# Youncy-Hu/MAGE

Hardware: AMD Instinct MI355X
Metric: generated frames/sec (64x64, 16-frame clips) (higher is better)
Workload: dtype bf16

## Files before the change

### include/mage_hip_ext.h

```cpp
#ifndef MAGE_HIP_EXT_H
#define MAGE_HIP_EXT_H

#include "mage_hip.h"

#ifdef __cplusplus
extern "C" {
#endif

int mage_token_stats(const float* logits, int64_t rows, int32_t K, int64_t ld, int64_t group, int64_t in_group_stride, int64_t in_off,
                     const int64_t* tokens, int64_t tok_group_stride, int64_t tok_off, float temperature, int32_t top_k, float top_p,
                     float* policy_logprob, float* policy_entropy, int32_t* kept, float* entropy, void* stream);

int mage_policy_loss(const float* logits, int64_t rows, int32_t K, int64_t ld, const int64_t* tokens, const float* advantage, int64_t adv_div,
                     const float* behaviour_logprob, float temperature, int32_t top_k, float top_p, float clip_lo, float clip_hi,
                     float entropy_coef, float* row_loss, float* logprob, float* entropy, uint32_t* cut, float* summary, void* stream);
int mage_policy_loss_bwd(const float* logits, int64_t rows, int32_t K, int64_t ld, const int64_t* tokens, const float* advantage,
                         int64_t adv_div, const float* behaviour_logprob, const uint32_t* cut, float temperature, float clip_lo,
                         float clip_hi, float entropy_coef, const float* grad_out, void* dlogits, int32_t dl_dtype, void* stream);

int mage_policy_loss_anchored(const float* logits, int64_t rows, int32_t K, int64_t ld, const int64_t* tokens, const float* advantage,
                              int64_t adv_div, const float* behaviour_logprob, const float* reference_logprob, float temperature,
                              int32_t top_k, float top_p, float clip_lo, float clip_hi, float entropy_coef, float kl_coef, float* row_loss,
                              float* logprob, float* entropy, uint32_t* cut, float* kl, float* summary, void* stream);
int mage_policy_loss_anchored_bwd(const float* logits, int64_t rows, int32_t K, int64_t ld, const int64_t* tokens, const float* advantage,
                                  int64_t adv_div, const float* behaviour_logprob, const float* reference_logprob, const uint32_t* cut,
                                  float temperature, float clip_lo, float clip_hi, float entropy_coef, float kl_coef, const float* grad_out,
                                  void* dlogits, int32_t dl_dtype, void* stream);

int mage_sumsq(const float* g, int64_t n, double* out, void* stream);
int mage_adam_clipped(float* p, const float* g, float* m, float* v, int64_t n, float lr, float beta1, float beta2, float eps, int32_t step,
                      float grad_scale, const double* sumsq, float max_norm, float* norm_out, void* stream);

int mage_video_metrics(const float* video, int64_t video_clip_stride, const float* target, int64_t target_clip_stride, int64_t clips, int32_t T,
                       int32_t C, int32_t H, int32_t W, int64_t tgt_div, float data_range, float* mse, float* psnr, float* ssim, void* stream);

int mage_group_advantages(const float* frame_reward, int64_t groups, int32_t N, int32_t T, int32_t mode, float eps, float* reward,
                          float* advantage, void* stream);

int mage_frame_advantages(const float* frame_reward, int64_t groups, int32_t N, int32_t T, float gamma, int32_t mode, float eps, int32_t slots,
                          int32_t slot_off, float* returns, float* advantage, void* stream);

int mage_video_noise(const int64_t* seeds, int64_t B, int32_t C, int64_t hw, float* nchw, float* rows, void* stream);

int mage_guide_logits(const float* cond, const float* uncond, float* out, int64_t rows, int32_t K, int64_t ld, int64_t group,
                      int64_t in_group_stride, int64_t in_off, const float* scale, int64_t scale_div, void* stream);

int mage_preference_loss(const float* clip_logprob, const float* reference_logprob, int64_t clips, const int64_t* pairs, int64_t n_pairs,
                         float beta, float label_smoothing, int32_t mode, float* pair_loss, float* pair_margin, float* clip_coef,
                         float* summary, void* stream);

int mage_token_logprob_bwd(const float* logits, int64_t rows, int32_t K, int64_t ld, const int64_t* tokens, const float* weight,
                           int64_t weight_div, const float* grad_out, void* dlogits, int32_t dl_dtype, void* stream);

int mage_gemm_attn_fused_qkv(const mage_gemm_desc* desc, int32_t axis, float scale, void* stream);
int mage_gemm_attn_fused_qkv_kernel_name(const mage_gemm_desc* desc, int32_t axis, char* buf, int32_t len);

int mage_apply_known_tokens(int64_t* tokens, int64_t rows, int64_t group, int64_t tok_group_stride, int64_t tok_off, const int64_t* known,
                            int64_t known_group_stride, int64_t known_off, int64_t known_clip_div, int32_t K, float* logprob,
                            float* policy_logprob, float* entropy, float* policy_entropy, int32_t* kept, void* stream);

int mage_policy_loss_masked(const float* logits, int64_t rows, int32_t K, int64_t ld, const int64_t* tokens, const float* advantage,
                            int64_t adv_div, const float* behaviour_logprob, const float* reference_logprob, float temperature, int32_t top_k,
                            float top_p, float clip_lo, float clip_hi, float entropy_coef, float kl_coef, float* row_loss, float* logprob,
                            float* entropy, uint32_t* cut, float* kl, float* summary, float* norm, const uint8_t* given, void* stream);
int mage_policy_loss_masked_bwd(const float* logits, int64_t rows, int32_t K, int64_t ld, const int64_t* tokens, const float* advantage,
                                int64_t adv_div, const float* behaviour_logprob, const float* reference_logprob, const uint32_t* cut,
                                float temperature, float clip_lo, float clip_hi, float entropy_coef, float kl_coef, const float* grad_out,
                                const float* norm, void* dlogits, int32_t dl_dtype, const uint8_t* given, void* stream);

int mage_policy_loss_grouped(const float* logits, int64_t rows, int32_t K, int64_t ld, const int64_t* tokens, const float* advantage,
                             int64_t adv_div, const float* behaviour_logprob, const float* reference_logprob, float temperature, int32_t top_k,
                             float top_p, float clip_lo, float clip_hi, float entropy_coef, float kl_coef, float* row_loss, float* logprob,
                             float* entropy, uint32_t* cut, float* kl, float* summary, float* norm, const uint8_t* given, int64_t ratio_div,
                             float* group_logratio, int32_t* group_count, void* stream);
int mage_policy_loss_grouped_bwd(const float* logits, int64_t rows, int32_t K, int64_t ld, const int64_t* tokens, const float* advantage,
                                 int64_t adv_div, const float* behaviour_logprob, const float* reference_logprob, const uint32_t* cut,
                                 float temperature, float clip_lo, float clip_hi, float entropy_coef, float kl_coef, const float* grad_out,
                                 const float* norm, void* dlogits, int32_t dl_dtype, const uint8_t* given, int64_t ratio_div,
                                 const float* group_logratio, void* stream);

int mage_token_logprob_bwd_masked(const float* logits, int64_t rows, int32_t K, int64_t ld, const int64_t* tokens, const float* weight,
                                  int64_t weight_div, const float* grad_out, void* dlogits, int32_t dl_dtype, const uint8_t* given,
                                  void* stream);

int mage_distill_loss(const float* logits, int64_t rows, int32_t K, int64_t ld, const float* teacher, int64_t ld_t, float temperature,
                      int32_t mode, const uint8_t* given, float* row_kl, float* summary, float* norm, void* stream);
int mage_distill_loss_bwd(const float* logits, int64_t rows, int32_t K, int64_t ld, const float* teacher, int64_t ld_t, float temperature,
                          int32_t mode, const uint8_t* given, const float* row_kl, const float* grad_out, const float* norm, void* dlogits,
                          int32_t dl_dtype, void* stream);
// ... 6 lines not shown
```

### mage_amd/_lib.py

```python
from __future__ import annotations

import ctypes as C
import os
from typing import Optional

_HERE = os.path.dirname(os.path.abspath(__file__))
LIB_PATH = os.environ.get("MAGE_HIP_LIB", os.path.join(_HERE, "lib", "libmage_hip.so"))

F32, BF16, BF16X3, F16X3, F16 = 0, 1, 2, 3, 4
ACT_NONE, ACT_RELU, ACT_QUICKGELU, ACT_GELU_ERF, ACT_TANH, ACT_QUICKGELU_GRAD = 0, 1, 2, 3, 4, 5
ABI_VERSION = 10

i32, i64, f32, vp = C.c_int32, C.c_int64, C.c_float, C.c_void_p


class GemmDesc(C.Structure):
    _fields_ = [
        ("dtype", i32), ("M", i32), ("N", i32), ("K", i32),
        ("A", vp), ("W", vp), ("Y", vp),
        ("lda", i32), ("ldy", i32), ("y_dtype", i32),
        ("out_h", i32), ("out_w", i32), ("in_h", i32), ("in_w", i32),
        ("a_img_stride", i32), ("a_off", i32),
        ("taps_h", i32), ("taps_w", i32), ("cin", i32), ("stride", i32),
        ("dy0", i32), ("dx0", i32), ("dys", i32), ("dxs", i32),
# ... 79 lines not shown
    "mage_colsum": (C.c_int, [vp, i64, i64, i32, vp, i32, vp]),
    "mage_row_sum": (C.c_int, [vp, i32, i64, i64, i32, vp, i32, vp]),
    "mage_sum_partials": (C.c_int, [vp, i64, i32, i64, vp, i32, vp]),
    "mage_layernorm_bwd": (C.c_int, [vp, vp, vp, i32, vp, vp, i32, i64, i32, f32, i32, vp, f32, C.c_uint64, vp]),
    "mage_act": (C.c_int, [vp, vp, i32, i64, i32, vp]),
    "mage_act_bwd": (C.c_int, [vp, vp, vp, i32, i64, i32, vp]),
    "mage_cross_entropy_bwd": (C.c_int, [vp, vp, i64, i32, vp, vp, i32, vp]),
    "mage_embedding_bwd": (C.c_int, [vp, vp, i32, vp, i64, i32, i32, i64, i64, i64, i64, vp, i64, vp]),
    "mage_group_rowsum": (C.c_int, [vp, i32, i64, i32, i64, i64, vp, i64, vp, i32, vp]),
    "mage_attention_bwd": (C.c_int, [C.POINTER(AttnDesc), vp, vp, vp, vp, i32, i32, i32, vp]),
    "mage_dropout": (C.c_int, [vp, i32, vp, i32, i64, f32, C.c_uint64, i32, vp]),
    "mage_dropout_add": (C.c_int, [vp, i32, vp, vp, vp, i64, f32, C.c_uint64, vp]),
    "mage_dropout_add_layernorm": (C.c_int, [vp, i32, vp, vp, vp, vp, vp, i32, i64, i32, f32, f32, C.c_uint64, vp]),
    "mage_adam": (C.c_int, [vp, vp, vp, vp, i64, f32, f32, f32, f32, i32, f32, vp]),
}

EXT_SIGNATURES = {
    "mage_token_stats": (C.c_int, [vp, i64, i32, i64, i64, i64, i64, vp, i64, i64, f32, i32, f32, vp, vp, vp, vp, vp]),
    "mage_policy_loss": (C.c_int, [vp, i64, i32, i64, vp, vp, i64, vp, f32, i32, f32, f32, f32, f32, vp, vp, vp, vp, vp, vp]),
    "mage_policy_loss_bwd": (C.c_int, [vp, i64, i32, i64, vp, vp, i64, vp, vp, f32, f32, f32, f32, vp, vp, i32, vp]),
    "mage_policy_loss_anchored": (C.c_int, [vp, i64, i32, i64, vp, vp, i64, vp, vp, f32, i32, f32, f32, f32, f32, f32, vp, vp, vp, vp, vp, vp, vp]),
    "mage_policy_loss_anchored_bwd": (C.c_int, [vp, i64, i32, i64, vp, vp, i64, vp, vp, vp, f32, f32, f32, f32, f32, vp, vp, i32, vp]),
    "mage_sumsq": (C.c_int, [vp, i64, vp, vp]),
    "mage_adam_clipped": (C.c_int, [vp, vp, vp, vp, i64, f32, f32, f32, f32, i32, f32, vp, f32, vp, vp]),
    "mage_video_metrics": (C.c_int, [vp, i64, vp, i64, i64, i32, i32, i32, i32, i64, f32, vp, vp, vp, vp]),
    "mage_group_advantages": (C.c_int, [vp, i64, i32, i32, i32, f32, vp, vp, vp]),
    "mage_frame_advantages": (C.c_int, [vp, i64, i32, i32, f32, i32, f32, i32, i32, vp, vp, vp]),
    "mage_video_noise": (C.c_int, [vp, i64, i32, i64, vp, vp, vp]),
    "mage_guide_logits": (C.c_int, [vp, vp, vp, i64, i32, i64, i64, i64, i64, vp, i64, vp]),
    "mage_preference_loss": (C.c_int, [vp, vp, i64, vp, i64, f32, f32, i32, vp, vp, vp, vp, vp]),
    "mage_token_logprob_bwd": (C.c_int, [vp, i64, i32, i64, vp, vp, i64, vp, vp, i32, vp]),
    "mage_gemm_attn_fused_qkv": (C.c_int, [C.POINTER(GemmDesc), i32, f32, vp]),
    "mage_gemm_attn_fused_qkv_kernel_name": (C.c_int, [C.POINTER(GemmDesc), i32, C.c_char_p, i32]),
    "mage_apply_known_tokens": (C.c_int, [vp, i64, i64, i64, i64, vp, i64, i64, i64, i32, vp, vp, vp, vp, vp, vp]),
    "mage_policy_loss_masked": (C.c_int, [vp, i64, i32, i64, vp, vp, i64, vp, vp, f32, i32, f32, f32, f32, f32, f32, vp, vp, vp, vp, vp, vp, vp,
                                          vp, vp]),
    "mage_policy_loss_masked_bwd": (C.c_int, [vp, i64, i32, i64, vp, vp, i64, vp, vp, vp, f32, f32, f32, f32, f32, vp, vp, vp, i32, vp, vp]),
    "mage_policy_loss_grouped": (C.c_int, [vp, i64, i32, i64, vp, vp, i64, vp, vp, f32, i32, f32, f32, f32, f32, f32, vp, vp, vp, vp, vp, vp, vp,
                                           vp, i64, vp, vp, vp]),
    "mage_policy_loss_grouped_bwd": (C.c_int, [vp, i64, i32, i64, vp, vp, i64, vp, vp, vp, f32, f32, f32, f32, f32, vp, vp, vp, i32, vp, i64, vp,
                                               vp]),
    "mage_token_logprob_bwd_masked": (C.c_int, [vp, i64, i32, i64, vp, vp, i64, vp, vp, i32, vp, vp]),
    "mage_distill_loss": (C.c_int, [vp, i64, i32, i64, vp, i64, f32, i32, vp, vp, vp, vp, vp]),
    "mage_distill_loss_bwd": (C.c_int, [vp, i64, i32, i64, vp, i64, f32, i32, vp, vp, vp, vp, vp, i32, vp]),
}

_lib: Optional[C.CDLL] = None
_inited_devices = set()


class MageHipError(RuntimeError):
    pass


def load(path: str = LIB_PATH) -> C.CDLL:
    global _lib
    if _lib is not None:
        return _lib
    if not os.path.exists(path):
        raise MageHipError(
            f"{path} not found: the HIP extension is not built. Run `python -c 'import __graft_entry__ as g; g.build()'` "
            f"(or `make -C mage_amd/csrc`). There is no CPU/PyTorch fallback for the MAGE product path.")
    import torch
    lib = C.CDLL(path)
    for name, (res, args) in {**SIGNATURES, **EXT_SIGNATURES}.items():
        fn = getattr(lib, name)
# ... 24 lines not shown
```

### mage_amd/config.py

```python
from __future__ import annotations

import contextlib
import dataclasses
import os
from typing import Iterator

__all__ = ["Config", "ENV", "get", "override", "lib_option", "lib_options", "lib_flag", "LIB_OPTIONS"]


@dataclasses.dataclass(frozen=True)
class Config:
    qk_fuse: bool = True
    ln_fold: bool = True
    stream_16bit: bool = True
    attn_split: bool = True
    frame_table: bool = True
    auto_graph: bool = True
    encode_split: bool = True
    decode_table: bool = True
    decode_split: bool = True
    decode_taps8: bool = True
    decode_resblock_fusion: bool = True
    decode_head_fusion: bool = True
    decode_phase_merge: bool = True
    decode_relu_fold: bool = True
    train_f32_branch: bool = False
    train_wgrad_transpose: bool = False
    train_emit: bool = True
    train_dual: bool = True
    train_taps: bool = True
    train_enc_split: bool = True


ENV = {
    "ln_fold": ("MAGE_NO_LN_FOLD", False),
    "qk_fuse": ("MAGE_NO_QK_FUSE", False),
    "stream_16bit": ("MAGE_STREAM_FP32", False),
    "attn_split": ("MAGE_ATTN_SPLIT_FP32", False),
    "frame_table": ("MAGE_NO_FRAME_TABLE", False),
    "auto_graph": ("MAGE_NO_AUTO_GRAPH", False),
    "encode_split": ("MAGE_ENCODE_FP32", False),
    "decode_table": ("MAGE_NO_DECODE_TABLE", False),
    "decode_split": ("MAGE_DECODE_FP32", False),
    "decode_taps8": ("MAGE_DECODE_NO_TAPS8", False),
    "decode_resblock_fusion": ("MAGE_DECODE_NO_RESBLOCK_FUSION", False),
    "decode_head_fusion": ("MAGE_DECODE_NO_HEAD_FUSION", False),
    "decode_phase_merge": ("MAGE_DECODE_NO_PHASE_MERGE", False),
    "decode_relu_fold": ("MAGE_DECODE_NO_RELU_FOLD", False),
    "train_f32_branch": ("MAGE_TRAIN_F32_BRANCH", True),
    "train_wgrad_transpose": ("MAGE_WGRAD_TRANSPOSE", True),
    "train_emit": ("MAGE_TRAIN_NO_EMIT", False),
    "train_dual": ("MAGE_TRAIN_NO_DUAL", False),
    "train_taps": ("MAGE_TRAIN_NO_TAPS", False),
    "train_enc_split": ("MAGE_TRAIN_ENC_FP32", False),
}

LIB_OPTIONS = ("gemm_no_4w", "gemm_no_4h", "gemm_4h_plain", "gemm4_train_forms", "gemm_no_8phase", "gemm_no_taps8", "gemm_no_narrow", "gemm_no_narrow_few", "gemm_no_small",
               "gemm_small_m", "gemm_stagger_groups", "gemm_stagger_percent", "gemm_stagger_forced",
               "gemm4_stagger_groups", "gemm4_stagger_percent", "attn_no_mfma", "attn_no_fewq", "vq_no_mfma", "conv_no_tile")


def _set(v) -> bool:
    return bool(v) and v != "0"


def _from_env() -> Config:
    kw = {}
    for field, (var, when_set) in ENV.items():
        if _set(os.environ.get(var)):
# ... 74 lines not shown
```

### mage_amd/modules/mage_model.py

```python
from __future__ import annotations

import contextlib
import ctypes
import gc
import math
from collections import OrderedDict
from math import exp
from typing import Dict, Optional, Tuple

import torch
from torch import nn

from .. import config, ops
from ..utils.util import default, instantiate_from_config, zero_module
from .vqvae_model import VectorQuantizedVAE, _Derived, _conv_w, _no_torch_forward, weights_frozen

__all__ = ["QuickGELU", "AxialAttentionBlock", "TransformerBlock", "MAEncoder", "TransformerTextEncoder", "BasicBlock",
           "ADAIN2D", "FlatAxialDecoder", "PIDControl", "MAGE"]

F32 = torch.float32
BF16 = torch.bfloat16
F16 = torch.float16
HALF_TYPES = (BF16, F16)

# ... 318 lines not shown
        B, Cc, H, W = x.shape
        xr = x.permute(0, 2, 3, 1).reshape(B * H * W, Cc).float().contiguous()
        yr = y.permute(0, 2, 3, 1).reshape(B * H * W, -1).float().contiguous()
        return self._run(xr, yr, B, H, W).view(B, H, W, Cc).permute(0, 3, 1, 2)


class FlatAxialDecoder(nn.Module):

    def __init__(self, in_channels, model_channels, out_channels, frames_length, layers, context_channels=None, use_cids=True,
                 dropout=0.1):
        super().__init__()
        self.in_channels, self.model_channels, self.out_channels = in_channels, model_channels, out_channels
        self.frames_length, self.layers = frames_length, layers
        self.in_linear = nn.Linear(in_channels, model_channels)
        context_channels = default(context_channels, in_channels)
        self.context_channels = context_channels
        self.context_linear = nn.Linear(context_channels, model_channels)
        scale = model_channels ** -0.5
        self.T_positional_embedding = nn.Parameter(scale * torch.randn(frames_length, 1, 1, model_channels))
        num_heads = model_channels // 32
        self.blocks = nn.ModuleList([AxialAttentionBlock(model_channels, num_heads, axial_dim=i % 3 + 1, dropout=dropout)
                                     for i in range(layers)])
        self.use_cids = use_cids
        if use_cids:
            self.out = nn.Linear(model_channels, out_channels)
        else:
            self.out = nn.Sequential(nn.GroupNorm(32, model_channels), nn.SiLU(),
                                     zero_module(nn.Conv3d(model_channels, out_channels, 1)))
        self.initialize_parameters()
        self.compute_dtype = F32
        self.split_kind = 0
        self.stream_bf16 = True
        self.qkv_fuse_tiles = 8
        self._derived = _Derived(self)

    def initialize_parameters(self):
        proj_std = (self.model_channels ** -0.5) * ((2 * self.layers) ** -0.5)
        attn_std = self.model_channels ** -0.5
        fc_std = (2 * self.model_channels) ** -0.5
        for block in self.blocks:
            nn.init.normal_(block.attn.in_proj_weight, std=attn_std)
            nn.init.normal_(block.attn.out_proj.weight, std=proj_std)
            nn.init.normal_(block.mlp.c_fc.weight, std=fc_std)
            nn.init.normal_(block.mlp.c_proj.weight, std=proj_std)

    def build_casual_attention_mask(self):
        mask = torch.empty(self.frames_length, self.frames_length)
        mask.fill_(float("-inf"))
        mask.triu_(1)
        return mask

    def _build(self):
        d: Dict[str, torch.Tensor] = {}
        _pack_linear(d, "in_linear", self.in_linear.weight, self.in_linear.bias)
        _pack_linear(d, "context_linear", self.context_linear.weight, self.context_linear.bias)
        if self.use_cids:
            _pack_linear(d, "out", self.out.weight, self.out.bias)
        else:
            d["gn.w"], d["gn.b"] = self.out[0].weight.float().contiguous(), self.out[0].bias.float().contiguous()
            w = self.out[2].weight.float().reshape(self.out_channels, self.model_channels)
            n8 = (self.out_channels + 7) // 8 * 8
            wp = torch.zeros(n8, self.model_channels, device=w.device)
            wp[:self.out_channels] = w
            bp = torch.zeros(n8, device=w.device)
            bp[:self.out_channels] = self.out[2].bias.float()
            _pack_linear(d, "out", wp, bp)
# ... 11 lines not shown
        return d

    def _fold(self, dt, B: int, hw: int) -> bool:
        return (dt in HALF_TYPES and (B * hw) % 256 == 0 and self.model_channels % 256 == 0 and config.get().ln_fold)

    def _stream_bf16(self) -> bool:
        return getattr(self, "stream_bf16", True) and config.get().stream_16bit

    def _ln_linear(self, d, p, lin, xn, xb, ln, y, *, M, N, **kw):
        Cc, name = self.model_channels, f"{p}.{lin}"
        if ln is None:
            return ops.gemm(xn, _wdt(d, name, self.compute_dtype), y, M=M, N=N, K=Cc, lda=Cc, ldy=N, bias=d[name + ".b"], **kw)
        lnw, lns = self._ln_fold_w(d, p, lin, xb.dtype)
        return ops.gemm(xb, lnw, y, M=M, N=N, K=Cc, lda=Cc, ldy=N, bias=d[name + ".lnc"], ln_colsum=lns, **ln, **kw)

    @staticmethod
    def _ln_fold_w(d, p, lin, dt):
        if dt == BF16:
            return d[f"{p}.{lin}.lnw"], d[f"{p}.{lin}.lns"]
        kw_, ks_ = f"{p}.{lin}.lnw.f16", f"{p}.{lin}.lns.f16"
        if kw_ not in d:
            ln = "ln_1" if lin == "in_proj" else "ln_2"
            wq = (d[f"{p}.{lin}.f32"] * d[f"{p}.{ln}.w"][None, :]).to(F16)
            d[kw_], d[ks_] = wq, wq.float().sum(dim=1).contiguous()
        return d[kw_], d[ks_]

    def _qkv_fuse(self, xb, M: int, hh: int, ww: int, stats_rows: bool, cache) -> bool:
        Cc = self.model_channels
        if not (stats_rows and cache is None and hh == 16 and ww == 16 and self.use_cids and config.get().qk_fuse):
            return False
        if Cc % 256 or not 256 <= Cc <= 1024 or M % 256 or (M + 8) * Cc * 2 >= 2 ** 32:
            return False
        return (M // 256) * (Cc // 128) >= getattr(self, "qkv_fuse_tiles", 8) * torch.cuda.get_device_properties(xb.device).multi_processor_count

    def _qkv_fuse_w(self, d, p, dt):
        sfx = ".f16" if dt == F16 else ""
        if f"{p}.in_proj.qkv.w{sfx}" not in d:
            lnw, lns = self._ln_fold_w(d, p, "in_proj", dt)
            self._qkv_fuse_pack(d, p, lnw, lns, sfx)
        q = f"{p}.in_proj.qkv."
        return dict(w=d[q + "w" + sfx], s=d[q + "s" + sfx], c=d[q + "c"])

    def _qkv_fuse_pack(self, d, p, lnw, lns, sfx: str) -> None:
        idx = ops.qkv_pack_rows(self.model_channels, lnw.device)
        d[f"{p}.in_proj.qkv.w{sfx}"], d[f"{p}.in_proj.qkv.s{sfx}"] = lnw[idx].contiguous(), lns[idx].contiguous()
        d[f"{p}.in_proj.qkv.c"] = d[f"{p}.in_proj.lnc"][idx].contiguous()

    def _stats_inline(self, xb, M: int) -> bool:
        Cc = self.model_channels
        return all(ops.gemm_is_small(xb, M, n, Cc) for n in (Cc, 2 * Cc, 3 * Cc, 4 * Cc))

    @torch.no_grad()
    def _run(self, motion: torch.Tensor, imgs: torch.Tensor, *, B: int, hh: int, ww: int) -> torch.Tensor:
        L = self.frames_length
        run = self._pass_split if self._split_on() else self._pass
        return run(motion, imgs, B=B, hh=hh, ww=ww, p0=0, P=L, nf=L - 1, cache=None)

    def _inc_begin(self, B: int, hh: int, ww: int) -> dict:
        return {"B": B, "hh": hh, "ww": ww, "kv": {}, "p": 0}

    @torch.no_grad()
    def _inc_step(self, st: dict, motion: Optional[torch.Tensor], imgs: torch.Tensor, nf: int = 1) -> torch.Tensor:
        p0 = st["p"]
        P = nf + 1 if motion is not None else nf
        assert self.use_cids and nf >= 1 and (p0 == 0) == (motion is not None) and p0 + P <= self.frames_length
        run = self._pass_split if self._split_on() else self._pass
# ... 47 lines not shown
        if split:
            return self._lin_s(xa, d, "out", logits, M=rows, N=self.out_channels, K=Cc, out_w=nf * hw, a_img_stride=P * hw, a_off=(P - nf) * hw)
        return _linear(xa, d, "out", logits, dt, M=rows, N=self.out_channels, K=Cc, out_w=nf * hw, a_img_stride=P * hw, a_off=(P - nf) * hw)

    def _pass(self, motion, imgs, *, B: int, hh: int, ww: int, p0: int, P: int, nf: int, cache: Optional[dict],
              nh: Optional[int] = None) -> torch.Tensor:
        d = self._derived.get(self._build)
        dt, Cc, L = self.compute_dtype, self.model_channels, self.frames_length
        dev = (imgs.tokens if isinstance(imgs, FrameTokens) else imgs).device
        hw = hh * ww
        M = B * P * hw
        fold = self._fold(dt, B, hw)
        sb = fold and self._stream_bf16()
        xb = part = stats = None
        if fold:
            xb = torch.empty(M, Cc, device=dev, dtype=dt)
            part = torch.empty(Cc // 64, M, 2, device=dev, dtype=F32)
            stats = torch.empty(M, 2, device=dev, dtype=F32)
        inl = fold and self._stats_inline(xb, M)
        ln = None if not fold else dict(ln_part=part, ln_eps=1e-5) if inl else dict(ln_stats=stats)
        ln0 = dict(ln_stats=stats) if sb else None
        x = xb if sb else torch.empty(M, Cc, device=dev, dtype=F32)
        res = dict(residual=x, ldr=Cc)
        if fold:
            res["ln_part"] = part
            if not sb:
                res.update(y2=xb, ldy2=Cc)
        self._embed(d, x, motion, imgs, B=B, hw=hw, P=P, nf=nf, tp=d["tpos"][p0:])
        if sb:
            ops.row_stats(xb, 1e-5, stats)
        xn = torch.empty(M, Cc, device=dev, dtype=dt)
        qkv = torch.empty(M, 3 * Cc, device=dev, dtype=dt)
        ao = torch.empty(M, Cc, device=dev, dtype=dt)
        hdn = torch.empty(M, 4 * Cc, device=dev, dtype=dt)
        geo = [self._axial_geo(a, B, hh, ww, P, p0, cached=cache is not None, q_cached=cache is not None) for a in range(3)]
        fuse = self._qkv_fuse(xb, M, hh, ww, fold and not inl, cache)
        for i in range(self.layers):
            p = f"b{i}"
            ln1 = ln if i else ln0
            if ln1 is None:
                ops.layernorm(x, d[p + ".ln_1.w"], d[p + ".ln_1.b"], xn, 1e-5)
            if fuse and i % 3:
                f = self._qkv_fuse_w(d, p, dt)
                ops.gemm_attn_fused_qkv(xb, f["w"], ao, axis=i % 3, M=M, C_=Cc, K=Cc, lda=Cc, ldy=Cc, bias=f["c"], ln_stats=stats, ln_colsum=f["s"])
            elif i % 3 == 0 and cache is not None:
                if p0 == 0:
                    cache[i] = torch.empty(B * L * hw, 3 * Cc, device=dev, dtype=dt)
                kv = cache[i]
                self._ln_linear(d, p, "in_proj", xn, xb, ln1, kv, M=M, N=3 * Cc, out_w=P * hw, y_img_stride=L * hw, y_off=p0 * hw)
                q = kv[p0 * hw:]
            else:
                q = kv = qkv
                self._ln_linear(d, p, "in_proj", xn, xb, ln1, qkv, M=M, N=3 * Cc)
            if not (fuse and i % 3):
                ops.attention(q, kv[:, Cc:], kv[:, 2 * Cc:], ao, ldq=3 * Cc, ldk=3 * Cc, ldv=3 * Cc, ldo=Cc, **geo[i % 3])
            _linear(ao, d, p + ".out_proj", x, dt, M=M, N=Cc, K=Cc, **res)
            if fold and not inl:
                ops.ln_stats(part, Cc, 1e-5, stats)
            if ln is None:
                ops.layernorm(x, d[p + ".ln_2.w"], d[p + ".ln_2.b"], xn, 1e-5)
            self._ln_linear(d, p, "c_fc", xn, xb, ln, hdn, M=M, N=4 * Cc, act=ops.ACT_QUICKGELU)
            if i < self.layers - 1:
                _linear(hdn, d, p + ".c_proj", x, dt, M=M, N=Cc, K=4 * Cc, **res)
                if fold and not inl:
                    ops.ln_stats(part, Cc, 1e-5, stats)
            else:
                if self.use_cids and dt != F32:
                    xa = xn
                else:
                    xa = torch.empty(M, Cc, device=dev, dtype=F32) if sb else x
                _linear(hdn, d, p + ".c_proj", xa, dt, M=M, N=Cc, K=4 * Cc, residual=x, ldr=Cc)
        return self._head(d, xa, B=B, hw=hw, P=P, nf=nf if nh is None else nh)

    def _split_on(self) -> bool:
        return bool(self.split_kind) and self.compute_dtype == F32 and self.model_channels % 64 == 0

    def _warm_split(self) -> None:
        if not self._split_on():
            return
        d = self._derived.get(self._build)
        names = ["in_linear", "context_linear"] + (["out"] if self.use_cids else [])
        for i in range(self.layers):
            names += [f"b{i}.in_proj", f"b{i}.out_proj", f"b{i}.c_fc", f"b{i}.c_proj"]
        for n in names:
            _wsplit(d, n, self.split_kind)

    def _attn_split(self) -> bool:
        return (self.split_kind == ops.F16X3 and self.frames_length <= 32 and (self.model_channels // 32) % 2 == 0
                and config.get().attn_split)

    def _taps_ok(self, rows: int) -> bool:
        return self.model_channels % 256 == 0 and rows % 256 == 0 and self.in_channels % 64 == 0 and self.context_channels % 64 == 0

# ... 1597 lines not shown
```

### mage_amd/ops.py

```python
from __future__ import annotations

import ctypes as C
from typing import Optional

import torch

from . import _lib
from ._lib import ACT_GELU_ERF, ACT_NONE, ACT_QUICKGELU, ACT_QUICKGELU_GRAD, ACT_RELU, ACT_TANH, BF16, BF16X3, F16, F16X3, F32, AttnDesc, GemmDesc

__all__ = ["gemm", "layernorm", "attention", "embedding", "table_conv", "split_rows", "vq_prepare", "vq_nearest", "argmax", "cross_entropy",
           "conv_in", "conv_out", "convt_fold_tanh", "row_affine", "groupnorm_silu", "groupnorm_act", "reparam_kl", "mse", "check_device_errors", "graph_events_supported", "transpose", "row_sum", "sum_partials", "layernorm_bwd", "dropout_add_layernorm", "act", "act_bwd", "cross_entropy_bwd", "embedding_bwd", "group_rowsum", "attention_bwd", "dropout", "adam", "adam_clipped", "sumsq", "bn_train_stats", "bn_apply", "bn_backward", "convt_unfold_tanh_bwd", "maxpool2", "upsample2", "relu", "cast", "adain", "add_scaled_rowvec",
           "token_logprob", "clip_scores", "video_metrics", "group_advantages", "frame_advantages", "policy_loss", "policy_loss_bwd", "preference_loss", "token_logprob_bwd", "distill_loss", "distill_loss_bwd", "split", "split_empty", "split_dtype", "PROFILE", "F32", "BF16", "F16", "BF16X3", "F16X3", "ACT_NONE", "ACT_RELU", "ACT_QUICKGELU", "ACT_GELU_ERF", "ACT_TANH", "tdtype", "code"]


def code(t: torch.Tensor) -> int:
    if t.dtype == torch.float32:
        return F32
    if t.dtype == torch.bfloat16:
        return BF16
    if t.dtype == torch.float16:
        return F16
    raise TypeError(f"unsupported dtype {t.dtype}")


# ... 253 lines not shown
                        y_off: int = 0):
    l, s = _dev(a)
    assert w.dtype == a.dtype and y.dtype == a.dtype, (w.dtype, y.dtype)
    out_w = M if out_w is None else out_w
    d = GemmDesc()
    d.dtype, d.M, d.N, d.K = code(a), M, 3 * C_, K
    d.A, d.W, d.Y = a.data_ptr(), w.data_ptr(), _p(y)
    d.lda, d.ldy, d.y_dtype = lda, ldy, code(y)
    d.out_h, d.out_w, d.in_h, d.in_w = 1, out_w, 1, out_w
    d.a_img_stride, d.a_off = out_w, a_off
    d.taps_h, d.taps_w, d.cin, d.stride = 1, 1, K, 1
    d.dys, d.dxs = 1, 1
    d.y_img_stride = out_w if y_img_stride is None else y_img_stride
    d.y_mul_y, d.y_mul_x, d.y_off = out_w, 1, y_off
    d.bias, d.ln_stats, d.ln_colsum = _p(bias), _p(ln_stats), _p(ln_colsum)
    d.n_split = 1
    sc = float(32 ** -0.5 if scale is None else scale)
    ev = None
    if PROFILE.enabled:
        buf = C.create_string_buffer(256)
        _lib.check(l.mage_gemm_attn_fused_qkv_kernel_name(C.byref(d), axis, buf, len(buf)), l)
        key = buf.value.decode()
        if PROFILE.wants(key):
            ev = PROFILE.begin()
    _lib.check(l.mage_gemm_attn_fused_qkv(C.byref(d), axis, sc, s), l)
    if ev is not None:
        es = a.element_size()
        nb = float(M) * K * es + 3.0 * C_ * K * es + float(M) * C_ * y.element_size()
        fl = 2.0 * M * 3 * C_ * K + 6.0 * M * 16 * C_
        PROFILE.end(key, ev, fl, nb)
    return y


def gemm_is_small(a: torch.Tensor, M: int, N: int, K: int) -> bool:
    l, _ = _dev(a)
    r = l.mage_gemm_is_small(M, N, K)
    if r < 0:
        _lib.check(r, l)
    return r == 1


def _gemm_split(l, s, a, w, y, *, M, N, K, lda, ldy, out_h, out_w, in_h, in_w, a_img_stride, a_off, taps_h, taps_w, cin, y_img_stride, y_mul_y,
                y_mul_x, y_off, bias, act, rowadd, rowadd_div, rowadd_mod, residual, ldr, ldw, split_kind, y_split):
    sd = split_dtype(split_kind)
    assert a.dtype == sd and w.dtype == sd and (y.dtype == sd if y_split else y.dtype == torch.float32), (a.dtype, w.dtype, y.dtype)
    out_w = M if out_w is None else out_w
    in_h = out_h if in_h is None else in_h
    in_w = out_w if in_w is None else in_w
    d = GemmDesc()
    d.dtype, d.M, d.N, d.K = split_kind, M, N, K
    d.A, d.W, d.Y = a.data_ptr(), w.data_ptr(), y.data_ptr()
    d.lda, d.ldy, d.y_dtype = lda, ldy, (split_kind if y_split else F32)
    d.out_h, d.out_w, d.in_h, d.in_w = out_h, out_w, in_h, in_w
    d.a_img_stride = in_h * in_w if a_img_stride is None else a_img_stride
    d.a_off = a_off
    d.taps_h, d.taps_w, d.cin, d.stride = taps_h, taps_w, (K // (taps_h * taps_w) if cin is None else cin), 1
    d.dy0, d.dx0, d.dys, d.dxs = 0, 0, 1, 1
    d.y_img_stride = out_h * out_w if y_img_stride is None else y_img_stride
    d.y_mul_y = out_w if y_mul_y is None else y_mul_y
    d.y_mul_x, d.y_off = y_mul_x, y_off
    d.bias, d.act = _p(bias), act
    d.rowadd, d.rowadd_div, d.rowadd_mod = _p(rowadd), rowadd_div, rowadd_mod
    d.residual, d.ldr, d.res_dtype = _p(residual), ldr, F32
    d.ldw, d.n_split = ldw, 1
    if PROFILE.enabled:
        key = _kernel_name(l, d)
# ... 1016 lines not shown
```

Baseline: 6043.

## Fuse transformer MLP (fc, QuickGELU, proj) into one persistent HIP kernel

Adds a persistent MFMA kernel that runs both MLP linears for C=512. The LayerNorm-folded c_fc output, with QuickGELU applied, stays in registers as the input to c_proj, so the 4C hidden activation is never written to or read from global memory. Weights for each 32-wide hidden chunk are streamed through LDS by direct global-to-LDS DMA and double-buffered. The residual add and the next LayerNorm's partial statistics are produced in the epilogue. It only runs for bf16/f16 with 512 channels and enough row tiles per CU, and the hand-scheduled inline assembly adds correctness and maintenance risk.

```diff
diff --git a/include/mage_hip_ext.h b/include/mage_hip_ext.h
--- a/include/mage_hip_ext.h
+++ b/include/mage_hip_ext.h
@@ -55,6 +55,13 @@
 int mage_gemm_attn_fused_qkv(const mage_gemm_desc* desc, int32_t axis, float scale, void* stream);
 int mage_gemm_attn_fused_qkv_kernel_name(const mage_gemm_desc* desc, int32_t axis, char* buf, int32_t len);
 
+int mage_mlp_fused(int32_t dtype, int32_t w_dtype, int32_t y_dtype, int64_t M, int32_t C, const void* x, int64_t ldx, int64_t a_off, void* y, int64_t ldy,
+                   int64_t y_off, const void* w1, int64_t ldw1, const float* c1, const float* s1, const float* ln_stats, const void* w2, int64_t ldw2,
+                   const float* b2, float* ln_part, int64_t ln_part_rows, void* stream);
+int mage_mlp_fused_kernel_name(int32_t dtype, int32_t w_dtype, int32_t y_dtype, int64_t M, int32_t C, const void* x, int64_t ldx, int64_t a_off, void* y,
+                               int64_t ldy, int64_t y_off, const void* w1, int64_t ldw1, const float* c1, const float* s1, const float* ln_stats,
+                               const void* w2, int64_t ldw2, const float* b2, float* ln_part, int64_t ln_part_rows, char* buf, int32_t len);
+
 int mage_apply_known_tokens(int64_t* tokens, int64_t rows, int64_t group, int64_t tok_group_stride, int64_t tok_off, const int64_t* known,
                             int64_t known_group_stride, int64_t known_off, int64_t known_clip_div, int32_t K, float* logprob,
                             float* policy_logprob, float* entropy, float* policy_entropy, int32_t* kept, void* stream);
diff --git a/mage_amd/_lib.py b/mage_amd/_lib.py
--- a/mage_amd/_lib.py
+++ b/mage_amd/_lib.py
@@ -135,6 +135,9 @@
     "mage_token_logprob_bwd": (C.c_int, [vp, i64, i32, i64, vp, vp, i64, vp, vp, i32, vp]),
     "mage_gemm_attn_fused_qkv": (C.c_int, [C.POINTER(GemmDesc), i32, f32, vp]),
     "mage_gemm_attn_fused_qkv_kernel_name": (C.c_int, [C.POINTER(GemmDesc), i32, C.c_char_p, i32]),
+    "mage_mlp_fused": (C.c_int, [i32, i32, i32, i64, i32, vp, i64, i64, vp, i64, i64, vp, i64, vp, vp, vp, vp, i64, vp, vp, i64, vp]),
+    "mage_mlp_fused_kernel_name": (C.c_int, [i32, i32, i32, i64, i32, vp, i64, i64, vp, i64, i64, vp, i64, vp, vp, vp, vp, i64, vp, vp, i64,
+                                             C.c_char_p, i32]),
     "mage_apply_known_tokens": (C.c_int, [vp, i64, i64, i64, i64, vp, i64, i64, i64, i32, vp, vp, vp, vp, vp, vp]),
     "mage_policy_loss_masked": (C.c_int, [vp, i64, i32, i64, vp, vp, i64, vp, vp, f32, i32, f32, f32, f32, f32, f32, vp, vp, vp, vp, vp, vp, vp,
                                           vp, vp]),
diff --git a/mage_amd/config.py b/mage_amd/config.py
--- a/mage_amd/config.py
+++ b/mage_amd/config.py
@@ -11,6 +11,7 @@
 @dataclasses.dataclass(frozen=True)
 class Config:
     qk_fuse: bool = True
+    mlp_fuse: bool = True
     ln_fold: bool = True
     stream_16bit: bool = True
     attn_split: bool = True
@@ -35,6 +36,7 @@
 ENV = {
     "ln_fold": ("MAGE_NO_LN_FOLD", False),
     "qk_fuse": ("MAGE_NO_QK_FUSE", False),
+    "mlp_fuse": ("MAGE_NO_MLP_FUSE", False),
     "stream_16bit": ("MAGE_STREAM_FP32", False),
     "attn_split": ("MAGE_ATTN_SPLIT_FP32", False),
     "frame_table": ("MAGE_NO_FRAME_TABLE", False),
diff --git a/mage_amd/csrc/gemm4m.hip b/mage_amd/csrc/gemm4m.hip
--- /dev/null
+++ b/mage_amd/csrc/gemm4m.hip
@@ -0,0 +1,349 @@
+#include "gemm_shared.h"
+#include "gemm4_regs.h"
+
+namespace {
+
+struct Gemm4mArgs {
+    const void* X;
+    void* Y;
+    const void* W1;
+    const void* W2;
+    const float* c1;
+    const float* s1;
+    const float* stats;
+    const float* b2;
+    float* ln_part;
+    long ln_part_rows;
+    int M, ldx, ldy, ldw1, ldw2, a_off, y_off, ntiles;
+};
+
+constexpr int M_C = 512, M_HID = 2048, M_NCH = M_HID / 32;
+constexpr int M_STG = 32768, M_W2OFF = 2 * M_STG, M_COFF = 4 * M_STG, M_SOFF = M_COFF + M_HID * 4, M_STGOFF = M_SOFF + M_HID * 4;
+constexpr int M_LDS = M_STGOFF + 4 * 4096;
+
+#ifndef MAGE4M_XPRE
+#define MAGE4M_XPRE 1
+#endif
+
+__device__ __forceinline__ void m_dma(unsigned lds, unsigned voff, const char* base) {
+    asm volatile("s_mov_b32 m0, %0\n\ts_nop 0\n\tglobal_load_lds_dwordx4 %1, %2" ::"s"(lds), "v"(voff), "s"(base) : "memory");
+}
+template <bool ZERO, bool CLOB, bool HF>
+__device__ __forceinline__ void m_mfma1(f32x4& acc, const u32x4& w, const u32x4& x) {
+#define M_MFMA1(OP)                                                                                              \
+    do {                                                                                                         \
+        if constexpr (ZERO && CLOB) asm volatile(OP " %0, %1, %2, 0" : "=&v"(acc) : "v"(w), "v"(x) : G4_ALL_ACC); \
+        else if constexpr (ZERO) asm volatile(OP " %0, %1, %2, 0" : "=&v"(acc) : "v"(w), "v"(x));                 \
+        else if constexpr (CLOB) asm volatile(OP " %0, %1, %2, %0" : "+v"(acc) : "v"(w), "v"(x) : G4_ALL_ACC);    \
+        else asm volatile(OP " %0, %1, %2, %0" : "+v"(acc) : "v"(w), "v"(x));                                     \
+    } while (0)
+    if constexpr (HF) M_MFMA1("v_mfma_f32_16x16x32_f16");
+    else M_MFMA1("v_mfma_f32_16x16x32_bf16");
+#undef M_MFMA1
+}
+constexpr int m_wait_imm(int vm) { return (((vm >> 4) & 3) << 14) | (vm & 15) | 0x70; }
+
+template <bool HF, bool LNP>
+__global__ __launch_bounds__(256) void gemm4m_kernel(const Gemm4mArgs g) {
+    typedef std::conditional_t<HF, f16_t, unsigned short> HT;
+    extern __shared__ __attribute__((aligned(16))) char smem[];
+    g4_claim_accumulators();
+    const int tid = threadIdx.x;
+    const int lane = tid & 63;
+    const int wave = __builtin_amdgcn_readfirstlane(tid >> 6);
+    const int l15 = lane & 15, grp = lane >> 4;
+    const unsigned smem_addr = (unsigned)(uintptr_t)(__attribute__((address_space(3))) char*)smem;
+
+    const int lr = lane >> 3, lp = lane & 7;
+    unsigned voffW1[2];
+#pragma unroll
+    for (int h = 0; h < 2; ++h)
+        voffW1[h] = (unsigned)((8 * (lr >> 2) + (lr & 3)) * g.ldw1 * 2 + ((lp ^ ((h * 4 + (lr >> 1)) & 7)) << 4));
+    const unsigned voffW2 = (unsigned)((lane >> 2) * g.ldw2 * 2 + (((lane & 3) ^ ((4 - (lane >> 4)) & 3)) << 4));
+    auto dma_w1 = [&](int stage, int c, int u) __attribute__((always_inline)) {
+        const int sl = 2 * wave + (u >> 2), u4 = u & 3;
+        const char* base = (const char*)g.W1 + (long)(32 * c + 16 * (u4 & 1) + 4 * (u4 >> 1)) * g.ldw1 * 2 + sl * 128;
+        m_dma(smem_addr + stage * M_STG + sl * 4096 + u4 * 1024, voffW1[u4 & 1], base);
+    };
+    auto dma_w2 = [&](int stage, int c, int u) __attribute__((always_inline)) {
+        const int nb = 8 * wave + u;
+        const char* base = (const char*)g.W2 + (long)(nb * 16) * g.ldw2 * 2 + c * 64;
+        m_dma(smem_addr + M_W2OFF + stage * M_STG + nb * 1024, voffW2, base);
+    };
+
+    const int rsw = (l15 >> 1) & 7;
+    const int w1_off = l15 * 128, w1_pc[2] = {((grp + 0) ^ rsw) * 16, ((grp + 4) ^ rsw) * 16};
+    const int w2_off = M_W2OFF + l15 * 64 + ((grp ^ ((4 - (l15 >> 2)) & 3)) << 4);
+    u32x4 wf[2][4];
+    auto rd_w1 = [&](int buf, int stage, int b, int j) __attribute__((always_inline)) {
+        const int ks = 2 * b + (j >> 1), t = j & 1;
+        wf[buf][j] = *(const u32x4*)(smem + stage * M_STG + (ks >> 1) * 4096 + t * 2048 + w1_off + w1_pc[ks & 1]);
+    };
+    auto rd_w2 = [&](int buf, int stage, int b, int j) __attribute__((always_inline)) {
+        wf[buf][j] = *(const u32x4*)(smem + stage * M_STG + (4 * b + j) * 1024 + w2_off);
+    };
+
+    u32x4 xf[2][16];
+    f32x4 hacc[2][2][2];
+    u32x4 hpk[2];
+    f32x4 sv, cv;
+    float mean[2], rstd[2];
+    const unsigned xoff = (unsigned)((l15 * g.ldx + 8 * grp) * 2);
+    auto load_x = [&](int tile, int mt0, int mt1) __attribute__((always_inline)) {
+#pragma unroll
+        for (int mt = mt0; mt < mt1; ++mt) {
+            const char* xp = (const char*)g.X + ((long)tile * 128 + wave * 32 + mt * 16 + g.a_off) * g.ldx * 2;
+#pragma unroll
+            for (int ks = 0; ks < 16; ++ks) xf[mt][ks] = *(const u32x4*)(xp + ks * 64 + xoff);
+        }
+    };
+    auto fence = [&]() __attribute__((always_inline)) { __builtin_amdgcn_sched_barrier(0); };
+    auto wait_barrier = [&]() __attribute__((always_inline)) {
+        __builtin_amdgcn_s_waitcnt(m_wait_imm(8));
+        ring_barrier();
+        fence();
+    };
+    float eu[4];
+    auto act_op = [&](auto PAR_, auto G_, auto K_) __attribute__((always_inline)) {
+        constexpr int PAR = decltype(PAR_)::value, G = decltype(G_)::value, K = decltype(K_)::value;
+        constexpr int t = G >> 1, mt = G & 1, a = K >> 2, j = K & 3;
+        float v = hacc[PAR][mt][t][j];
+        if constexpr (a == 0) asm volatile("v_fma_f32 %0, -%1, %2, %0" : "+v"(v) : "v"(mean[mt]), "v"(sv[j]));
+        else if constexpr (a == 1) asm volatile("v_fma_f32 %0, %1, %0, %2" : "+v"(v) : "v"(rstd[mt]), "v"(cv[j]));
+        else if constexpr (a == 2) asm volatile("v_mul_f32 %0, 0xc01d265f, %1" : "=v"(eu[j]) : "v"(v));
+        else if constexpr (a == 3) asm volatile("v_exp_f32 %0, %0" : "+v"(eu[j]));
+        else if constexpr (a == 4) asm volatile("v_add_f32 %0, 1.0, %0" : "+v"(eu[j]));
+        else if constexpr (a == 5) asm volatile("v_rcp_f32 %0, %0" : "+v"(eu[j]));
+        else asm volatile("v_mul_f32 %0, %0, %1" : "+v"(v) : "v"(eu[j]));
+        if constexpr (a < 2 || a == 6) hacc[PAR][mt][t][j] = v;
+    };
+    auto pack_op = [&](auto PAR_, auto I_) __attribute__((always_inline)) {
+        constexpr int PAR = decltype(PAR_)::value, I = decltype(I_)::value, mt = I >> 2, w = I & 3;
+        const float a0 = hacc[PAR][mt][w >> 1][(w & 1) * 2], a1 = hacc[PAR][mt][w >> 1][(w & 1) * 2 + 1];
+        unsigned r;
+        if constexpr (HF) asm volatile("v_cvt_pk_f16_f32 %0, %1, %2" : "=v"(r) : "v"(a0), "v"(a1));
+        else asm volatile("v_cvt_pk_bf16_f32 %0, %1, %2" : "=v"(r) : "v"(a0), "v"(a1));
+        hpk[mt][w] = r;
+    };
+    auto consts_rd = [&](int c, int t, int i) __attribute__((always_inline)) {
+        const char* p = smem + (i ? M_COFF : M_SOFF) + (32 * c + 8 * grp + 4 * t) * 4;
+        if (i) cv = *(const f32x4*)p;
+        else sv = *(const f32x4*)p;
+    };
+
+    auto phase_a = [&](auto PAR_, auto PACK_, int c) __attribute__((always_inline)) {
+        constexpr int PAR = decltype(PAR_)::value;
+        constexpr bool PACK = decltype(PACK_)::value;
+        g4_for<64>([&](auto i_) {
+            constexpr int i = decltype(i_)::value, b = i >> 3, k = i & 7, j = k >> 1, mt = k & 1, ks = 2 * b + (j >> 1), t = j & 1;
+            m_mfma1<ks == 0, k == 0, HF>(hacc[PAR][mt][t], wf[b & 1][j], xf[mt][ks]);
+            fence();
+            if constexpr (k < 4 && b < 7) rd_w1((b + 1) & 1, PAR, b + 1, k);
+            if constexpr (k < 4 && b == 7 && PACK) rd_w2(0, PAR ^ 1, 0, k);
+            if constexpr (PACK && i >= 8 && i < 16) pack_op(std::integral_constant<int, PAR ^ 1>{}, std::integral_constant<int, i - 8>{});
+            if constexpr (b >= 4 && (k == 4 || k == 6)) dma_w2(PAR, c, (b - 4) * 2 + (k == 6));
+            fence();
+            if constexpr (i == 31) wait_barrier();
+        });
+    };
+    auto phase_b = [&](auto PAR_, auto ZERO_, int c) __attribute__((always_inline)) {
+        constexpr int PAR = decltype(PAR_)::value;
+        constexpr bool ZERO = decltype(ZERO_)::value;
+        g4_for<64>([&](auto i_) {
+            constexpr int i = decltype(i_)::value, b = i >> 3, k = i & 7, j = k >> 1, mt = k & 1, nb = 4 * b + j;
+            g4_mfma<mt * 32 + nb, ZERO, k == 0, HF>(wf[b & 1][j], hpk[mt]);
+            fence();
+            if constexpr (i == 23 || i == 24) consts_rd(c, 1, i - 23);
+            if constexpr (i == 56 || i == 57) consts_rd((c + 1) & (M_NCH - 1), 0, i - 56);
+            if constexpr (k < 4 && b < 7) rd_w2((b + 1) & 1, PAR ^ 1, b + 1, k);
+            if constexpr (k < 4 && b == 7) rd_w1(0, PAR ^ 1, 0, k);
+            if constexpr (i >= 4 && i < 60) {
+                constexpr int o = 2 * (i - 4);
+                fence();
+                act_op(PAR_, std::integral_constant<int, o / 28>{}, std::integral_constant<int, o % 28>{});
+                act_op(PAR_, std::integral_constant<int, (o + 1) / 28>{}, std::integral_constant<int, (o + 1) % 28>{});
+            }
+            if constexpr (b >= 4 && (k == 4 || k == 6)) dma_w1(PAR, (c + 2) & (M_NCH - 1), (b - 4) * 2 + (k == 6));
+            fence();
+            if constexpr (i == 31) wait_barrier();
+        });
+    };
+    typedef std::integral_constant<int, 0> I0;
+    typedef std::integral_constant<int, 1> I1;
+
+    for (int i = tid; i < M_HID / 4; i += 256) {
+        ((f32x4*)(smem + M_COFF))[i] = ((const f32x4*)g.c1)[i];
+        ((f32x4*)(smem + M_SOFF))[i] = ((const f32x4*)g.s1)[i];
+    }
+#pragma unroll
+    for (int u = 0; u < 8; ++u) dma_w1(0, 0, u);
+#pragma unroll
+    for (int u = 0; u < 8; ++u) dma_w1(1, 1, u);
+    load_x(blockIdx.x, 0, 2);
+    __builtin_amdgcn_s_waitcnt(0x0070);
+    ring_barrier();
+    fence();
+
+    for (int tile = blockIdx.x; tile < g.ntiles; tile += gridDim.x) {
+        MAGE_DASSERT(tile >= 0 && tile < g.ntiles);
+        const int m0 = tile * 128 + wave * 32;
+#pragma unroll
+        for (int mt = 0; mt < 2; ++mt) {
+            const float2 st = *(const float2*)((const char*)(g.stats + 2 * (long)(m0 + mt * 16)) + (unsigned)(l15 * 8));
+            mean[mt] = st.x;
+            rstd[mt] = st.y;
+        }
+        g4_for<4>([&](auto j_) { rd_w1(0, 0, 0, decltype(j_)::value); });
+        fence();
+        phase_a(I0{}, std::false_type{}, 0);
+        consts_rd(0, 0, 0);
+        consts_rd(0, 0, 1);
+        asm volatile("s_nop 15" ::: "memory");
+        fence();
+        g4_for<56>([&](auto k_) { act_op(I0{}, std::integral_constant<int, decltype(k_)::value / 28>{}, std::integral_constant<int, decltype(k_)::value % 28>{}); });
+        fence();
+        consts_rd(0, 1, 0);
+        consts_rd(0, 1, 1);
+        fence();
+        g4_for<56>([&](auto k_) { act_op(I0{}, std::integral_constant<int, 2 + decltype(k_)::value / 28>{}, std::integral_constant<int, decltype(k_)::value % 28>{}); });
+        fence();
+        consts_rd(1, 0, 0);
+        consts_rd(1, 0, 1);
+        fence();
+        wait_barrier();
+#pragma unroll
+        for (int u = 0; u < 8; ++u) dma_w1(0, 2, u);
+        g4_for<4>([&](auto j_) { rd_w1(0, 1, 0, decltype(j_)::value); });
+        fence();
+        phase_a(I1{}, std::true_type{}, 1);
+        phase_b(I1{}, std::true_type{}, 1);
+        for (int c = 2; c < M_NCH; c += 2) {
+            phase_a(I0{}, std::true_type{}, c);
+            phase_b(I0{}, std::false_type{}, c);
+            phase_a(I1{}, std::true_type{}, c + 1);
+            phase_b(I1{}, std::false_type{}, c + 1);
+        }
+        asm volatile("s_nop 15" ::: "memory");
+        fence();
+        g4_for<8>([&](auto i_) { pack_op(I1{}, i_); });
+        fence();
+        wait_barrier();
+        g4_for<4>([&](auto j_) { rd_w2(0, 1, 0, decltype(j_)::value); });
+        fence();
+        const int ntile = tile + (int)gridDim.x < g.ntiles ? tile + (int)gridDim.x : tile;
+        load_x(ntile, 0, MAGE4M_XPRE);
+        fence();
+        asm volatile("s_nop 1" ::: "memory");
+        g4_for<64>([&](auto i_) {
+            constexpr int i = decltype(i_)::value, b = i >> 3, k = i & 7, j = k >> 1, mt = k & 1, nb = 4 * b + j;
+            g4_mfma<mt * 32 + nb, false, k == 0, HF>(wf[b & 1][j], hpk[mt]);
+            fence();
+            if constexpr (k < 4 && b < 7) rd_w2((b + 1) & 1, 1, b + 1, k);
+            fence();
+        });
+        asm volatile("s_nop 15\n\ts_nop 7" ::: "memory");
+        fence();
+        {
+            mage_gemm_desc d = {};
+            d.M = g.M;
+            d.N = M_C;
+            d.out_h = 1;
+            d.out_w = g.M;
+            d.y_mul_x = 1;
+            d.y_off = g.y_off;
+            d.ldy = g.ldy;
+            d.Y = g.Y;
+            d.residual = (const HT*)g.X + (long)(g.a_off - g.y_off) * g.ldx;
+            d.ldr = g.ldx;
+            d.ln_part = g.ln_part;
+            d.ln_part_rows = g.ln_part_rows;
+            char* stg = smem + M_STGOFF + wave * 4096;
+            int lane_e = lane;
+            asm volatile("" : "+v"(lane_e));
+            const int grp_e = lane_e >> 4;
+            g4_for<8>([&](auto sl_) {
+                constexpr int sl = decltype(sl_)::value;
+                f32x4 acc[2][4], biasm[4];
+#pragma unroll
+                for (int nt = 0; nt < 4; ++nt) biasm[nt] = *(const f32x4*)(g.b2 + sl * 64 + nt * 16 + grp_e * 4);
+                g4_for<8>([&](auto q_) {
+                    constexpr int q = decltype(q_)::value, mt = q >> 2, nt = q & 3;
+                    acc[mt][nt] = g4_acc_read<mt * 32 + 4 * sl + nt, q == 0>();
+                });
+                epilogue_lean<MAGE_ACT_NONE, HT, 2, false, LNP ? LN_PRODUCE : LN_NONE, 0, HT, true>(d, biasm, acc, m0, sl * 64, lane_e, g.M, stg, 0);
+                fence();
+            });
+        }
+        fence();
+        load_x(ntile, MAGE4M_XPRE, 2);
+        fence();
+    }
+    __builtin_amdgcn_s_waitcnt(0x0070);
+}
+
+template <bool HF, bool LNP>
+int launch4m(const Gemm4mArgs& a, hipStream_t s, int n_cu) {
+    const int grid = a.ntiles >= n_cu ? n_cu : a.ntiles;
+    return mage_gemm_launch<gemm4m_kernel<HF, LNP>>(grid, 256, M_LDS, s, a);
+}
+
+}
+
+extern "C" int mage_mlp_fused(int32_t dtype, int32_t w_dtype, int32_t y_dtype, int64_t M, int32_t C, const void* x, int64_t ldx, int64_t a_off, void* y, int64_t ldy, int64_t y_off,
+                              const void* w1, int64_t ldw1, const float* c1, const float* s1, const float* ln_stats, const void* w2, int64_t ldw2,
+                              const float* b2, float* ln_part, int64_t ln_part_rows, void* stream) {
+    MAGE_CHECK_ARG(dtype == MAGE_BF16 || dtype == MAGE_F16, "mage_mlp_fused: bf16 or f16 rows and weights (dtype %d)", (int)dtype);
+    MAGE_CHECK_ARG(w_dtype == dtype && y_dtype == dtype, "mage_mlp_fused: weights (dtype %d) and output rows (dtype %d) must have the type of x (%d)",
+                   (int)w_dtype, (int)y_dtype, (int)dtype);
+    MAGE_CHECK_ARG(C == M_C, "mage_mlp_fused: C=%d: the kernel is built for C = 512 (hidden = 2048)", (int)C);
+    MAGE_CHECK_ARG(M > 0 && M % 128 == 0, "mage_mlp_fused: M=%ld must be a positive multiple of 128 (whole row tiles)", (long)M);
+    MAGE_CHECK_ARG(x && y && w1 && c1 && s1 && ln_stats && w2 && b2, "mage_mlp_fused: x, y, w1, c1, s1, ln_stats, w2, b2 must be given");
+    MAGE_CHECK_ARG(ldx >= C && ldy >= C && ldx % 8 == 0 && ldy % 8 == 0, "mage_mlp_fused: ldx=%ld, ldy=%ld must be multiples of 8 and >= C", (long)ldx,
+                   (long)ldy);
+    MAGE_CHECK_ARG(ldw1 >= C && ldw2 >= 4 * C && ldw1 % 8 == 0 && ldw2 % 8 == 0, "mage_mlp_fused: ldw1=%ld >= C, ldw2=%ld >= 4C, multiples of 8",
+                   (long)ldw1, (long)ldw2);
+    MAGE_CHECK_ARG((((uintptr_t)x | (uintptr_t)y | (uintptr_t)w1 | (uintptr_t)w2 | (uintptr_t)c1 | (uintptr_t)s1 | (uintptr_t)b2) & 15) == 0 &&
+                       (((uintptr_t)ln_stats | (uintptr_t)ln_part) & 7) == 0,
+                   "mage_mlp_fused: rows, weights and vectors must be 16-byte aligned, ln_stats and ln_part 8-byte aligned");
+    MAGE_CHECK_ARG(a_off >= 0 && y_off >= 0 && (x != y || a_off == y_off), "mage_mlp_fused: row offsets a_off=%ld, y_off=%ld (equal when in place)",
+                   (long)a_off, (long)y_off);
+    MAGE_CHECK_ARG(!ln_part || ln_part_rows >= M + y_off, "mage_mlp_fused: ln_part_rows=%ld must cover the output rows", (long)ln_part_rows);
+    MAGE_CHECK_ARG((M + a_off) * ldx < (1L << 31) && (M + y_off) * ldy < (1L << 31) && 2048 * ldw1 * 2 < (1L << 31) && 512 * ldw2 * 2 < (1L << 31),
+                   "mage_mlp_fused: operands beyond the kernel's 32-bit row arithmetic");
+    Gemm4mArgs a;
+    a.X = x;
+    a.Y = y;
+    a.W1 = w1;
+    a.W2 = w2;
+    a.c1 = c1;
+    a.s1 = s1;
+    a.stats = ln_stats;
+    a.b2 = b2;
+    a.ln_part = ln_part;
+    a.ln_part_rows = ln_part_rows;
+    a.M = (int)M;
+    a.ldx = (int)ldx;
+    a.ldy = (int)ldy;
+    a.ldw1 = (int)ldw1;
+    a.ldw2 = (int)ldw2;
+    a.a_off = (int)a_off;
+    a.y_off = (int)y_off;
+    a.ntiles = (int)(M / 128);
+    hipStream_t s = (hipStream_t)stream;
+    const int n_cu = mage_gemm_cu_count();
+    const bool hf = dtype == MAGE_F16;
+    if (ln_part) return hf ? launch4m<true, true>(a, s, n_cu) : launch4m<false, true>(a, s, n_cu);
+    return hf ? launch4m<true, false>(a, s, n_cu) : launch4m<false, false>(a, s, n_cu);
+}
+
+extern "C" int mage_mlp_fused_kernel_name(int32_t dtype, int32_t w_dtype, int32_t y_dtype, int64_t M, int32_t C, const void* x, int64_t ldx, int64_t a_off, void* y, int64_t ldy,
+                                          int64_t y_off, const void* w1, int64_t ldw1, const float* c1, const float* s1, const float* ln_stats,
+                                          const void* w2, int64_t ldw2, const float* b2, float* ln_part, int64_t ln_part_rows, char* buf, int32_t len) {
+    MAGE_CHECK_ARG(buf != nullptr && len > 0, "mage_mlp_fused_kernel_name: no buffer");
+    const void* kernel = nullptr;
+    mage_gemm_plan = &kernel;
+    const int r = mage_mlp_fused(dtype, w_dtype, y_dtype, M, C, x, ldx, a_off, y, ldy, y_off, w1, ldw1, c1, s1, ln_stats, w2, ldw2, b2, ln_part, ln_part_rows, nullptr);
+    mage_gemm_plan = nullptr;
+    if (r != MAGE_OK) return r;
+    return mage_kernel_symbol_name(kernel, buf, len, "mage_mlp_fused_kernel_name");
+}
diff --git a/mage_amd/modules/mage_model.py b/mage_amd/modules/mage_model.py
--- a/mage_amd/modules/mage_model.py
+++ b/mage_amd/modules/mage_model.py
@@ -374,6 +374,7 @@
         self.split_kind = 0
         self.stream_bf16 = True
         self.qkv_fuse_tiles = 8
+        self.mlp_fuse_tiles = 8
         self._derived = _Derived(self)
 
     def initialize_parameters(self):
@@ -451,6 +452,13 @@
         if Cc % 256 or not 256 <= Cc <= 1024 or M % 256 or (M + 8) * Cc * 2 >= 2 ** 32:
             return False
         return (M // 256) * (Cc // 128) >= getattr(self, "qkv_fuse_tiles", 8) * torch.cuda.get_device_properties(xb.device).multi_processor_count
+
+    def _mlp_fuse(self, xb, M: int, stats_rows: bool, sb: bool) -> bool:
+        if not (stats_rows and sb and self.use_cids and self.model_channels == 512 and config.get().mlp_fuse):
+            return False
+        if M % 128 or M * 512 >= 2 ** 31:
+            return False
+        return M // 128 >= getattr(self, "mlp_fuse_tiles", 8) * torch.cuda.get_device_properties(xb.device).multi_processor_count
 
     def _qkv_fuse_w(self, d, p, dt):
         sfx = ".f16" if dt == F16 else ""
@@ -564,9 +572,10 @@
         xn = torch.empty(M, Cc, device=dev, dtype=dt)
         qkv = torch.empty(M, 3 * Cc, device=dev, dtype=dt)
         ao = torch.empty(M, Cc, device=dev, dtype=dt)
-        hdn = torch.empty(M, 4 * Cc, device=dev, dtype=dt)
         geo = [self._axial_geo(a, B, hh, ww, P, p0, cached=cache is not None, q_cached=cache is not None) for a in range(3)]
         fuse = self._qkv_fuse(xb, M, hh, ww, fold and not inl, cache)
+        mfuse = self._mlp_fuse(xb, M, fold and not inl, sb)
+        hdn = None if mfuse else torch.empty(M, 4 * Cc, device=dev, dtype=dt)
         for i in range(self.layers):
             p = f"b{i}"
             ln1 = ln if i else ln0
@@ -591,6 +600,16 @@
                 ops.ln_stats(part, Cc, 1e-5, stats)
             if ln is None:
                 ops.layernorm(x, d[p + ".ln_2.w"], d[p + ".ln_2.b"], xn, 1e-5)
+            if mfuse:
+                lnw, lns = self._ln_fold_w(d, p, "c_fc", dt)
+                last = i == self.layers - 1
+                ops.mlp_fused(xb, xn if last else xb, M=M, C_=Cc, w1=lnw, c1=d[p + ".c_fc.lnc"], s1=lns, ln_stats=stats,
+                              w2=_wdt(d, p + ".c_proj", dt), b2=d[p + ".c_proj.b"], ln_part=None if last else part)
+                if last:
+                    xa = xn
+                else:
+                    ops.ln_stats(part, Cc, 1e-5, stats)
+                continue
             self._ln_linear(d, p, "c_fc", xn, xb, ln, hdn, M=M, N=4 * Cc, act=ops.ACT_QUICKGELU)
             if i < self.layers - 1:
                 _linear(hdn, d, p + ".c_proj", x, dt, M=M, N=Cc, K=4 * Cc, **res)
diff --git a/mage_amd/ops.py b/mage_amd/ops.py
--- a/mage_amd/ops.py
+++ b/mage_amd/ops.py
@@ -309,6 +309,33 @@
     return y
 
 
+def mlp_fused(x: torch.Tensor, y: torch.Tensor, *, M: int, C_: int, w1: torch.Tensor, c1, s1, ln_stats, w2: torch.Tensor, b2, ln_part=None,
+              ldx: Optional[int] = None, ldy: Optional[int] = None, a_off: int = 0, y_off: int = 0, ldw1: Optional[int] = None,
+              ldw2: Optional[int] = None):
+    l, s = _dev(x)
+    ldx, ldy = C_ if ldx is None else ldx, C_ if ldy is None else ldy
+    ldw1, ldw2 = C_ if ldw1 is None else ldw1, 4 * C_ if ldw2 is None else ldw2
+    lpr = 0
+    if ln_part is not None:
+        assert ln_part.dtype == torch.float32 and ln_part.dim() == 3 and ln_part.shape[2] == 2 and ln_part.is_contiguous(), tuple(ln_part.shape)
+        lpr = ln_part.shape[1]
+    args = (code(x), code(w1), code(y), M, C_, x.data_ptr(), ldx, a_off, y.data_ptr(), ldy, y_off, w1.data_ptr(), ldw1, _p(c1), _p(s1), _p(ln_stats),
+            w2.data_ptr(), ldw2, _p(b2), _p(ln_part), lpr)
+    ev = None
+    if PROFILE.enabled:
+        buf = C.create_string_buffer(256)
+        _lib.check(l.mage_mlp_fused_kernel_name(*args, buf, len(buf)), l)
+        key = buf.value.decode()
+        if PROFILE.wants(key):
+            ev = PROFILE.begin()
+    _lib.check(l.mage_mlp_fused(*args, s), l)
+    if ev is not None:
+        es = x.element_size()
+        nb = 2.0 * M * C_ * es + 8.0 * C_ * C_ * es + (float(M) * (C_ // 64) * 8 if ln_part is not None else 0.0)
+        PROFILE.end(key, ev, 2.0 * M * C_ * 4 * C_ * 2, nb)
+    return y
+
+
 def gemm_is_small(a: torch.Tensor, M: int, N: int, K: int) -> bool:
     l, _ = _dev(a)
     r = l.mage_gemm_is_small(M, N, K)
```

Result: faster. 6488 (median of 6 runs) (+7.4%).
